# kaylode/vehicle-counting

Hardware: AMD Instinct MI355X
Metric: end-to-end frames/sec (detect+NMS+ReID+track), YOLOv5s 640px (higher is better)
Workload: dtype bf16; 1 GPU; YOLOv5s 640x640 single camera stream per GPU, bf16 convs (BASELINE.json configs[1]); workload_id=s640-bf16, clip_frames=512, objects=12, num_classes=80, detection_injection=False, weights=seeded synthetic (no checkpoints available), streams=1, ranks=1, counts_allgather_via=vc_allgather_counts (RCCL, C ABI), tracked_rows=155352, tracker=device-resident (one kernel per batch, no host round trip per frame)

## Files before the change

### vehicle-counting_amd/csrc/bneck_fused.hip

```cpp
#include <algorithm>

#include "kernels.h"
#include "conv_launch.h"

namespace vc {

typedef float f32x4b __attribute__((ext_vector_type(4)));
typedef float f32x2b __attribute__((ext_vector_type(2)));
typedef __bf16 bf16x8b __attribute__((ext_vector_type(8)));
typedef __bf16 bf16x2b __attribute__((ext_vector_type(2)));
typedef unsigned int u32x2b __attribute__((ext_vector_type(2)));
union ChunkB { uint4 u; bf16x8b h; };

#define BN_TH 8
#define BN_TW 16
#define BN_RW (BN_TW + 2)
#define BN_NH ((BN_TH + 2) * BN_RW)
#define BN_NT ((BN_NH + 15) / 16)
#define BN_NP BN_NH
#define BN_NW 8
#define BN_PLANE (BN_NP * 64)

__device__ __forceinline__ int bn_addr(int px, int chunk) { return (px * 4 + (chunk ^ ((px >> 1) & 2))) * 16; }
__device__ __forceinline__ f32x2b bn_sigmoid2(f32x2b x) {
// ... 6 lines not shown
    const f32x2b d = (f32x2b){__builtin_amdgcn_exp2f(t.x), __builtin_amdgcn_exp2f(t.y)} + (f32x2b){1.0f, 1.0f};
    return x * (f32x2b){__builtin_amdgcn_rcpf(d.x), __builtin_amdgcn_rcpf(d.y)};
}

struct BnArgs {
    const uint4 *w1, *w2;
    const float *b1, *b2;
    int kw1, kw2;
    const uint16_t* x; int in_cs, in_co;
    uint16_t* y; int out_cs, out_co;
    int B, H, W, tiles_x, tiles_y, res;
    const uint4* w3; const float* b3; int kw3;
    const uint16_t* y2; int y2_cs;
    uint16_t* z; int z_cs, z_co;
    long long* dbg;
};

template <bool CV3>
__global__ __launch_bounds__(BN_NW * 64) void bneck_fused_kernel(const BnArgs a) {
    const bool RES = a.res != 0;
    if (a.dbg && threadIdx.x == 0) a.dbg[(size_t)blockIdx.x * 2] = wall_clock64();
    __shared__ uint4 bs[2][2 * BN_NP * 4];
    __shared__ uint4 w1s[2 * 4 * 64];
    __shared__ uint4 w2s[18 * 4 * 64];
    __shared__ uint4 w3s[CV3 ? 4 * 8 * 64 : 1];
    __shared__ float b3s[CV3 ? 128 : 4];
    static_assert(sizeof(bs) + sizeof(w1s) + sizeof(w2s) + sizeof(w3s) + sizeof(b3s) <= 160 * 1024, "static LDS of bneck_fused_kernel exceeds a CU's 160 KB");
    const int lane = threadIdx.x & 63, wave = threadIdx.x >> 6;
    const int col = lane & 15, kq = lane >> 4;
    constexpr int NT = BN_NW * 64;
    for (int i = threadIdx.x; i < 2 * 4 * 64; i += NT) {
        const int l = i & 63, ct = (i >> 6) & 3, s = i >> 8;
        w1s[i] = a.w1[(size_t)(ct * 16 + (l & 15)) * a.kw1 + 4 * s + (l >> 4)];
    }
    for (int i = threadIdx.x; i < 18 * 4 * 64; i += NT) {
        const int l = i & 63, ct = (i >> 6) & 3, s = i >> 8;
        w2s[i] = a.w2[(size_t)(ct * 16 + (l & 15)) * a.kw2 + 4 * s + (l >> 4)];
    }
    if constexpr (CV3) {
        for (int i = threadIdx.x; i < 4 * 8 * 64; i += NT) {
            const int l = i & 63, ct = (i >> 6) & 7, s = i >> 9;
            w3s[i] = a.w3[(size_t)(ct * 16 + (l & 15)) * a.kw3 + 4 * s + (l >> 4)];
        }
        if (threadIdx.x < 128) b3s[threadIdx.x] = a.b3[threadIdx.x];
    }
    const bool producer = wave >= 4;
    const int gw = wave & 3;
    float4 bv[4];
#pragma unroll
    for (int ct = 0; ct < 4; ++ct) bv[ct] = *(const float4*)((producer ? a.b1 : a.b2) + ct * 16 + kq * 4);
    const int ntiles = a.B * a.tiles_y * a.tiles_x;
    const int nk = (int)blockIdx.x < ntiles ? (ntiles - 1 - (int)blockIdx.x) / (int)gridDim.x + 1 : 0;
    const bool odd = (kq & 1) != 0;
    __syncthreads();

    uint4 yf[3][2], yn[3][2];
    auto load_y = [&](int t, uint4 (&dst)[3][2]) {
        const int tx = t % a.tiles_x, ty = (t / a.tiles_x) % a.tiles_y, b = t / (a.tiles_x * a.tiles_y);
#pragma unroll
        for (int j = 0; j < 3; ++j) {
            const int n = (gw * 3 + j) * 16 + col;
            const int ry = (n * 3641) >> 16, rx = n - ry * BN_RW;
            const int gy = ty * BN_TH - 1 + ry, gx = tx * BN_TW - 1 + rx;
            dst[j][0] = make_uint4(0u, 0u, 0u, 0u); dst[j][1] = dst[j][0];
            if (n < BN_NH && gy >= 0 && gy < a.H && gx >= 0 && gx < a.W) {
                const uint16_t* px = a.x + (((size_t)b * a.H + gy) * a.W + gx) * a.in_cs + a.in_co + kq * 8;
                dst[j][0] = *(const uint4*)px; dst[j][1] = *(const uint4*)(px + 32);
            }
        }
    };
    if (producer && nk > 0) load_y(blockIdx.x, yf);
    for (int k = 0; k <= nk; ++k) {
        if (producer) {
            if (k < nk) {
                const int t = blockIdx.x + k * gridDim.x;
                if (k + 1 < nk) load_y(t + gridDim.x, yn);
                const int tx = t % a.tiles_x, ty = (t / a.tiles_x) % a.tiles_y;
                char* bsb = (char*)bs[k & 1];
                f32x4b pacc[3][4];
#pragma unroll
                for (int j = 0; j < 3; ++j) {
                    ChunkB y0f, y1f;
                    y0f.u = yf[j][0]; y1f.u = yf[j][1];
#pragma unroll
                    for (int ct = 0; ct < 4; ++ct) {
                        ChunkB w0, w1;
                        w0.u = w1s[(0 * 4 + ct) * 64 + lane]; w1.u = w1s[(1 * 4 + ct) * 64 + lane];
                        pacc[j][ct] = __builtin_amdgcn_mfma_f32_16x16x32_bf16(w0.h, y0f.h, (f32x4b){0.f, 0.f, 0.f, 0.f}, 0, 0, 0);
                        pacc[j][ct] = __builtin_amdgcn_mfma_f32_16x16x32_bf16(w1.h, y1f.h, pacc[j][ct], 0, 0, 0);
                    }
                }
// ... 7 lines not shown
#pragma unroll
                    for (int ct = 0; ct < 4; ++ct) {
                        const f32x4b acc = pacc[j][ct];
                        const f32x2b lo = bn_silu2((f32x2b){acc[0], acc[1]} + (f32x2b){bv[ct].x, bv[ct].y});
                        const f32x2b hi = bn_silu2((f32x2b){acc[2], acc[3]} + (f32x2b){bv[ct].z, bv[ct].w});
                        const bf16x2b p0 = {(__bf16)lo.x, (__bf16)lo.y}, p1 = {(__bf16)hi.x, (__bf16)hi.y};
                        uint2 v = make_uint2(__builtin_bit_cast(uint32_t, p0), __builtin_bit_cast(uint32_t, p1));
                        if (!inimg) v = make_uint2(0u, 0u);
                        if (n < BN_NH) *(uint2*)(bsb + (ct >> 1) * BN_PLANE + bn_addr(n, (ct & 1) * 2 + (kq >> 1)) + (kq & 1) * 8) = v;
                    }
                }
#pragma unroll
                for (int j = 0; j < 3; ++j) { yf[j][0] = yn[j][0]; yf[j][1] = yn[j][1]; }
            }
        } else if (k >= 1) {
            const int t = blockIdx.x + (k - 1) * gridDim.x;
            const int tx = t % a.tiles_x, ty = (t / a.tiles_x) % a.tiles_y, b = t / (a.tiles_x * a.tiles_y);
            const int oy0 = ty * BN_TH, ox0 = tx * BN_TW;
            const char* bsb = (const char*)bs[(k - 1) & 1];
            uint2 rs[4][2] = {};
            if (RES) {
#pragma unroll
                for (int q = 0; q < 2; ++q) {
                    const int oy = oy0 + gw * 2 + q, ox = ox0 + col;
                    const bool ok = oy < a.H && ox < a.W;
                    const uint16_t* px = a.x + (((size_t)b * a.H + min(oy, a.H - 1)) * a.W + min(ox, a.W - 1)) * a.in_cs + a.in_co + kq * 4;
#pragma unroll
                    for (int ct = 0; ct < 4; ++ct) rs[ct][q] = ok ? *(const uint2*)(px + ct * 16) : make_uint2(0u, 0u);
                }
            }
            uint4 y2f[2][2];
// ... 112 lines not shown
                    for (int q = 0; q < 2; ++q) {
                        const f32x2b lo = bn_silu2((f32x2b){zacc[ct][q][0], zacc[ct][q][1]} + (f32x2b){b3.x, b3.y});
                        const f32x2b hi = bn_silu2((f32x2b){zacc[ct][q][2], zacc[ct][q][3]} + (f32x2b){b3.z, b3.w});
                        const bf16x2b p0 = {(__bf16)lo.x, (__bf16)lo.y}, p1 = {(__bf16)hi.x, (__bf16)hi.y};
                        P[q] = make_uint2(__builtin_bit_cast(uint32_t, p0), __builtin_bit_cast(uint32_t, p1));
                    }
                    const u32x2b sx = __builtin_amdgcn_permlane16_swap(P[0].x, P[1].x, false, false);
                    const u32x2b sy = __builtin_amdgcn_permlane16_swap(P[0].y, P[1].y, false, false);
                    const uint4 o4 = make_uint4(sx.x, sy.x, sx.y, sy.y);
                    const int oy = oy0 + gw * 2 + (odd ? 1 : 0), ox = ox0 + col;
                    if (oy < a.H && ox < a.W)
                        *(uint4*)(a.z + (((size_t)b * a.H + oy) * a.W + ox) * a.z_cs + a.z_co + ct * 16 + (kq & ~1) * 4) = o4;
                }
            }
        }
        __syncthreads();
    }
    if (a.dbg && threadIdx.x == 0) a.dbg[(size_t)blockIdx.x * 2 + 1] = wall_clock64();
}

bool bneck_fused_applicable(const ConvP& pm1, const ConvP& pm2) {
    if (!(pm1.prec == PREC_BF16 && pm1.kh == 1 && pm1.kw == 1 && pm1.sh == 1 && pm1.sw == 1 && pm1.ph == 0 && pm1.pw == 0 && pm1.Cin == 64 && pm1.Cout == 64 &&
          pm1.act == ACT_SILU && pm1.res_mode == RES_NONE && !pm1.out_f32 && pm1.split == 0))
        return false;
    if (!(pm2.prec == PREC_BF16 && pm2.kh == 3 && pm2.kw == 3 && pm2.sh == 1 && pm2.sw == 1 && pm2.ph == 1 && pm2.pw == 1 && pm2.Cin == 64 && pm2.Cout == 64 &&
          pm2.act == ACT_SILU && (pm2.res_mode == RES_NONE || pm2.res_mode == RES_AFTER_ACT) && !pm2.out_f32 && pm2.split == 0))
        return false;
    if (!(pm2.in == pm1.out && pm2.in_co == pm1.out_co && pm2.in_cs == pm1.out_cs && pm2.H == pm1.H && pm2.W == pm1.W && pm2.B == pm1.B)) return false;
    if (pm2.res_mode == RES_AFTER_ACT && !(pm2.res == pm1.in && pm2.res_co == pm1.in_co && pm2.res_cs == pm1.in_cs)) return false;
    if (pm2.out == pm1.in && pm2.out_co < pm1.in_co + 64 && pm1.in_co < pm2.out_co + 64) return false;
    return pm1.in_cs % 8 == 0 && pm1.in_co % 8 == 0 && pm2.out_cs % 8 == 0 && pm2.out_co % 8 == 0 && pm1.Kp >= 64 && pm2.Kp >= 576;
}
// ... 23 lines not shown
    a.y = nullptr;
    a.w3 = (const uint4*)p3.w; a.b3 = p3.bias; a.kw3 = p3.Kp / 8;
    a.y2 = (const uint16_t*)p3.in + p3.in_co + 64; a.y2_cs = p3.in_cs;
    a.z = (uint16_t*)p3.out; a.z_cs = p3.out_cs; a.z_co = p3.out_co;
    a.B = pm1.B; a.H = pm1.H; a.W = pm1.W;
    a.tiles_x = (a.W + BN_TW - 1) / BN_TW; a.tiles_y = (a.H + BN_TH - 1) / BN_TH;
    const int ntiles = a.B * a.tiles_x * a.tiles_y;
    int dev = 0, cus = 256;
    hipDeviceProp_t prop;
    if (hipGetDevice(&dev) == hipSuccess && hipGetDeviceProperties(&prop, dev) == hipSuccess) cus = prop.multiProcessorCount;
    a.res = pm2.res_mode == RES_AFTER_ACT ? 1 : 0;
    int grid = std::min(ntiles, bneck_grid_cap(cus));
    if (grid_cap > 0) grid = std::min(grid, grid_cap);
    static WgStamps stamps("VC_BN_DBG", "bneck cv3", 1024, 2, 0, 1);
    a.dbg = stamps.next(grid, ntiles, s);
    launch_timed(pm1, bneck_fused_kernel<true>, dim3(grid), dim3(BN_NW * 64), 0, s, a);
    VC_HIP(hipGetLastError());
    if (a.dbg) stamps.report(s, [](const long long*, int, int) {});
    return VC_OK;
}

int launch_bneck_fused(const ConvP& pm1, const ConvP& pm2, hipStream_t s, int grid_cap) {
    if (!bneck_fused_applicable(pm1, pm2)) return VC_ERR_ARG;
    BnArgs a{};
    a.w1 = (const uint4*)pm1.w; a.w2 = (const uint4*)pm2.w; a.b1 = pm1.bias; a.b2 = pm2.bias;
    a.kw1 = pm1.Kp / 8; a.kw2 = pm2.Kp / 8;
    a.x = (const uint16_t*)pm1.in; a.in_cs = pm1.in_cs; a.in_co = pm1.in_co;
    a.y = (uint16_t*)pm2.out; a.out_cs = pm2.out_cs; a.out_co = pm2.out_co;
    a.B = pm1.B; a.H = pm1.H; a.W = pm1.W;
    a.tiles_x = (a.W + BN_TW - 1) / BN_TW; a.tiles_y = (a.H + BN_TH - 1) / BN_TH;
    const int ntiles = a.B * a.tiles_x * a.tiles_y;
    static const int cus = [] {
        int dev = 0, n = 256;
        hipDeviceProp_t prop;
        if (hipGetDevice(&dev) == hipSuccess && hipGetDeviceProperties(&prop, dev) == hipSuccess) n = prop.multiProcessorCount;
        return n;
    }();
    int grid = std::min(ntiles, bneck_grid_cap(cus));
    if (grid_cap > 0) grid = std::min(grid, grid_cap);
    a.res = pm2.res_mode == RES_AFTER_ACT ? 1 : 0;
    static WgStamps stamps("VC_BN_DBG", "bneck", 1024, 2, 0, 1);
    a.dbg = stamps.next(grid, ntiles, s);
    launch_timed(pm1, bneck_fused_kernel<false>, dim3(grid), dim3(BN_NW * 64), 0, s, a);
    VC_HIP(hipGetLastError());
    if (a.dbg) stamps.report(s, [](const long long*, int, int) {});
    return VC_OK;
}

}
```

### vehicle-counting_amd/csrc/c3_fused.hip

```cpp
#include <algorithm>

#include "kernels.h"
#include "conv_launch.h"

namespace vc {

typedef float f32x4c __attribute__((ext_vector_type(4)));
typedef float f32x2c __attribute__((ext_vector_type(2)));
typedef __bf16 bf16x8c __attribute__((ext_vector_type(8)));
typedef __bf16 bf16x2c __attribute__((ext_vector_type(2)));
typedef unsigned int u32x2c __attribute__((ext_vector_type(2)));
union ChunkC { uint4 u; bf16x8c h; };

#define C3_TH 8
#define C3_TW 16
#define C3_RW (C3_TW + 2)
#define C3_NH ((C3_TH + 2) * C3_RW)
#define C3_NT ((C3_NH + 15) / 16)
#define C3_NP (C3_NT * 16)
#define C3_NW 4

__device__ __forceinline__ int c3_addr(int px, int chunk) { return (px * 4 + (chunk ^ ((px >> 1) & 2))) * 16; }
__device__ __forceinline__ f32x2c c3_silu2(f32x2c x) {
    const f32x2c t = x * (f32x2c){-1.442695040888963387f, -1.442695040888963387f};
// ... 6 lines not shown
    f32x2c hi = (f32x2c){a[2], a[3]} + (f32x2c){b.z, b.w};
    if constexpr (!NOTRANS) { lo = c3_silu2(lo); hi = c3_silu2(hi); }
    const bf16x2c p0 = {(__bf16)lo.x, (__bf16)lo.y}, p1 = {(__bf16)hi.x, (__bf16)hi.y};
    return make_uint2(__builtin_bit_cast(uint32_t, p0), __builtin_bit_cast(uint32_t, p1));
}

struct C3Args {
    const uint4 *w12, *wm1, *wm2, *w3;
    const float *b12, *bm1, *bm2, *b3;
    int kw12, kwm1, kwm2, kw3;
    const uint16_t* x; int in_cs, in_co;
    uint16_t* y; int out_cs, out_co;
    int B, H, W, tiles_x, tiles_y;
    int abl;
    long long* dbg;
};

template <bool DIAG>
__global__ __launch_bounds__(C3_NW * 64, 2) void c3_fused_kernel(const C3Args a) {
    const int abl = DIAG ? a.abl : 0;
    if (a.dbg && threadIdx.x == 0) a.dbg[(size_t)blockIdx.x * 2] = wall_clock64();
    __shared__ uint4 xa[2 * C3_NP * 4];
    __shared__ uint4 yb[C3_NP * 4];
    __shared__ uint4 yc[C3_TH * C3_TW * 4];
    __shared__ uint4 w12s[2 * 4 * 64], wm1s[2 * 64], wm2s[9 * 2 * 64], w3s[2 * 4 * 64];
    const int lane = threadIdx.x & 63, wave = threadIdx.x >> 6;
    const int col = lane & 15, kq = lane >> 4;
    constexpr int NT = C3_NW * 64;
    for (int i = threadIdx.x; i < 2 * 4 * 64; i += NT) {
        const int l = i & 63, ct = (i >> 6) & 3, s = i >> 8;
// ... 24 lines not shown
#pragma unroll
        for (int k = 0; k < NPRE; ++k) {
            const int i = threadIdx.x + k * NT;
            const int n = i >> 3, c = i & 7;
            const int ry = (n * 3641) >> 16, rx = n - ry * C3_RW;
            const int gy = y0 + ry, gx = x0 + rx;
            pre[k] = make_uint4(0u, 0u, 0u, 0u);
            if (n < C3_NH && gy >= 0 && gy < a.H && gx >= 0 && gx < a.W && !(abl & 2))
                pre[k] = *(const uint4*)(a.x + (((size_t)b * a.H + gy) * a.W + gx) * a.in_cs + a.in_co + c * 8);
        }
    };
    char* xab = (char*)xa;
    char* ybb = (char*)yb;
    char* ycb = (char*)yc;
    const bool odd = (kq & 1) != 0;
    if ((int)blockIdx.x < ntiles) fetch(blockIdx.x);
    for (int t = blockIdx.x; t < ntiles; t += gridDim.x) {
        const int tx = t % a.tiles_x, ty = (t / a.tiles_x) % a.tiles_y, b = t / (a.tiles_x * a.tiles_y);
        const int oy0 = ty * C3_TH, ox0 = tx * C3_TW;
#pragma unroll
        for (int k = 0; k < NPRE; ++k) {
            const int i = threadIdx.x + k * NT;
            const int n = i >> 3, c = i & 7;
            if (n < C3_NH) *(uint4*)(xab + (c >> 2) * (C3_NP * 64) + c3_addr(n, c & 3)) = pre[k];
        }
        __syncthreads();
        if (t + (int)gridDim.x < ntiles) fetch(t + gridDim.x);

        for (int pt = wave; pt < C3_NT && !(abl & 16); pt += C3_NW) {
            const int n = pt * 16 + col;
            ChunkC x0f, x1f;
            x0f.u = *(const uint4*)(xab + c3_addr(n, kq));
            x1f.u = *(const uint4*)(xab + C3_NP * 64 + c3_addr(n, kq));
            f32x4c acc[4];
#pragma unroll
            for (int ct = 0; ct < 4; ++ct) {
                ChunkC w0, w1;
                w0.u = w12s[(0 * 4 + ct) * 64 + lane]; w1.u = w12s[(1 * 4 + ct) * 64 + lane];
                acc[ct] = __builtin_amdgcn_mfma_f32_16x16x32_bf16(w0.h, x0f.h, (f32x4c){0.f, 0.f, 0.f, 0.f}, 0, 0, 0);
                acc[ct] = __builtin_amdgcn_mfma_f32_16x16x32_bf16(w1.h, x1f.h, acc[ct], 0, 0, 0);
            }
            const int ry = (n * 3641) >> 16, rx = n - ry * C3_RW;
// ... 86 lines not shown
                    acc[ct][q] = __builtin_amdgcn_mfma_f32_16x16x32_bf16(w1.h, yf[q].h, acc[ct][q], 0, 0, 0);
                }
            }
#pragma unroll
            for (int ct = 0; ct < 4; ++ct) {
                const uint2 P0 = act4(acc[ct][0], b3[ct]), P1 = act4(acc[ct][1], b3[ct]);
                const u32x2c sx = __builtin_amdgcn_permlane16_swap(P0.x, P1.x, false, false);
                const u32x2c sy = __builtin_amdgcn_permlane16_swap(P0.y, P1.y, false, false);
                const uint4 o4 = make_uint4(sx.x, sy.x, sx.y, sy.y);
                const int oy = oy0 + wave * 2 + (odd ? 1 : 0), ox = ox0 + col;
                if (oy < a.H && ox < a.W && !(abl & 4))
                    *(uint4*)(a.y + (((size_t)b * a.H + oy) * a.W + ox) * a.out_cs + a.out_co + ct * 16 + (kq & ~1) * 4) = o4;
            }
        }
    }
    if (a.dbg && threadIdx.x == 0) a.dbg[(size_t)blockIdx.x * 2 + 1] = wall_clock64();
}

bool c3_fused_applicable(const ConvP& p12, const ConvP& pm1, const ConvP& pm2, const ConvP& p3) {
    auto pw = [](const ConvP& p, int cin, int cout) {
        return p.prec == PREC_BF16 && p.kh == 1 && p.kw == 1 && p.sh == 1 && p.sw == 1 && p.ph == 0 && p.pw == 0 && p.Cin == cin && p.Cout == cout &&
               p.act == ACT_SILU && p.res_mode == RES_NONE && !p.out_f32;
    };
    if (!pw(p12, 64, 64) || p12.split != 32 || !pw(pm1, 32, 32) || pm1.split != 0 || !pw(p3, 64, 64) || p3.split != 0) return false;
    if (!(pm2.prec == PREC_BF16 && pm2.kh == 3 && pm2.kw == 3 && pm2.sh == 1 && pm2.sw == 1 && pm2.ph == 1 && pm2.pw == 1 && pm2.Cin == 32 && pm2.Cout == 32 &&
          pm2.act == ACT_SILU && pm2.res_mode == RES_AFTER_ACT && !pm2.out_f32 && pm2.split == 0))
        return false;
    const bool chain = pm1.in == p12.out && pm1.in_co == p12.out_co && pm2.in == pm1.out && pm2.in_co == pm1.out_co && pm2.res == p12.out && pm2.res_co == p12.out_co &&
                       pm2.out == p3.in && pm2.out_co == p3.in_co && p12.out2 == p3.in && p12.out2_co == p3.in_co + 32 && pm2.out_cs == p3.in_cs && p12.out2_cs == p3.in_cs;
    const bool shape = pm1.H == p12.H && pm2.H == p12.H && p3.H == p12.H && pm1.W == p12.W && pm2.W == p12.W && p3.W == p12.W && pm1.B == p12.B && p3.B == p12.B;
// ... 2 lines not shown

int launch_c3_fused(const ConvP& p12, const ConvP& pm1, const ConvP& pm2, const ConvP& p3, hipStream_t s, int grid_cap) {
    if (!c3_fused_applicable(p12, pm1, pm2, p3)) return VC_ERR_ARG;
    C3Args a{};
    a.w12 = (const uint4*)p12.w; a.wm1 = (const uint4*)pm1.w; a.wm2 = (const uint4*)pm2.w; a.w3 = (const uint4*)p3.w;
    a.b12 = p12.bias; a.bm1 = pm1.bias; a.bm2 = pm2.bias; a.b3 = p3.bias;
    a.kw12 = p12.Kp / 8; a.kwm1 = pm1.Kp / 8; a.kwm2 = pm2.Kp / 8; a.kw3 = p3.Kp / 8;
    a.x = (const uint16_t*)p12.in; a.in_cs = p12.in_cs; a.in_co = p12.in_co;
    a.y = (uint16_t*)p3.out; a.out_cs = p3.out_cs; a.out_co = p3.out_co;
    a.B = p12.B; a.H = p12.H; a.W = p12.W;
    a.tiles_x = (a.W + C3_TW - 1) / C3_TW; a.tiles_y = (a.H + C3_TH - 1) / C3_TH;
    const int ntiles = a.B * a.tiles_x * a.tiles_y;
    static const int slots_hw = resident_workgroups(c3_fused_kernel<false>, C3_NW * 64);
    int grid = std::min(ntiles, std::max(256, slots_hw - conv_slots_reserve() / 2));
    if (grid_cap > 0) grid = std::min(grid, grid_cap);
    a.abl = p12.ablate;
    static WgStamps stamps("VC_C3_DBG", "c3", 1024, 2, 0, 1);
    a.dbg = stamps.next(grid, ntiles, s);
    if (a.abl) launch_timed(p12, c3_fused_kernel<true>, dim3(grid), dim3(C3_NW * 64), 0, s, a);
    else launch_timed(p12, c3_fused_kernel<false>, dim3(grid), dim3(C3_NW * 64), 0, s, a);
    VC_HIP(hipGetLastError());
    if (a.dbg) stamps.report(s, [](const long long*, int, int) {});
    return VC_OK;
}

}
```

### vehicle-counting_amd/csrc/engine.h

```cpp
#pragma once
#include <chrono>
#include <condition_variable>
#include <deque>
#include <map>
#include <mutex>
#include <memory>
#include <string>
#include <vector>

#include "kernels.h"
#include "det_prep.h"
#include "host_stage.h"

namespace vc {

struct ConvParam {
    std::string name;
    int O = 0, I = 0, kh = 0, kw = 0;
    bool set = false;
    bool pair_stem = false;
    int fuse_a = -1, fuse_b = -1;
    int obj_of = -1;
    bool hidden = false;
    std::vector<float> w, b;
// ... 79 lines not shown
}

struct vc_render;

struct vc_engine {
    vc_engine_config cfg{};
    int prec = 0;
    int aux_prec = 0;
    float act_scale = 1.0f;
    hipStream_t stream = nullptr;
    hipStream_t dstream = nullptr;
    hipStream_t rstream = nullptr;
    hipStream_t hstream = nullptr;
    hipEvent_t ev_fork = nullptr, ev_join = nullptr;
    static constexpr unsigned kTileCtrPairs = 1024;
    unsigned* d_tile_ctr = nullptr;
    unsigned tile_ctr_seq = 0;
    unsigned tile_ctr_ring = kTileCtrPairs;
    int conv_slots = 0;
    void* d_zero = nullptr; size_t zero_bytes = 0; bool want_hc_count = false;
    hipEvent_t ev_det[2] = {nullptr, nullptr};
    hipEvent_t ev_reid[3] = {nullptr, nullptr, nullptr};
    bool finalized = false;
    struct Options { int c3_fused = 1, bneck_fused = 1, bneck_cv3 = 1, front_fused = 1, crop_per_pixel = 0, sparse_head = 1, ff_ablate = 0, c3_ablate = 0, reid_block_fused = 1, dyn_tiles = 1, head_side = 1, fuse_upsample = 1, sppf_sep = 1, fuse_s2_pw = 1, stem_direct = 1, embed_kept_only = 1; } opt;
    std::vector<void*> allocs;
    std::vector<void*> host_allocs;

    vc::Net yolo;
    int ch[5] = {0, 0, 0, 0, 0}, rep[4] = {0, 0, 0, 0};
    std::map<std::string, vc::View> ybuf;
    const vc::YoloPlan* last_plan = nullptr;
    std::vector<vc::ConvP> s2pw_folded;
    std::vector<std::pair<vc::View, vc::View>> up_folded;
    std::map<std::vector<int>, vc::YoloPlan> yolo_plans;
    std::map<std::pair<int, int>, vc::ReidPlan> reid_plans;
    uint8_t* d_frames = nullptr;
    size_t d_frames_bytes = 0;
    float* d_logits[3] = {nullptr, nullptr, nullptr};
    void* d_obj[3] = {nullptr, nullptr, nullptr};
// ... 116 lines not shown
    vc::ProfCat prof[VC_PROF_NCAT];
    hipEvent_t ev0 = nullptr, ev1 = nullptr;
    std::map<std::string, int> tuned;
    bool tuned_dirty = false;
    std::string op_log;
    double last_ms = 0;

    std::vector<float> inject_det;
    std::vector<int> inject_count;
    int inject_b = 0, inject_n = 0;
};

namespace vc {
int pack_and_upload(std::vector<void*>& allocs, ConvParam& p, int prec, float act_scale = 1.0f);
inline int dev_alloc(vc_engine* e, void** p, size_t bytes) { return dev_alloc(e->allocs, p, bytes); }
inline unsigned* tile_ctr_next(vc_engine* e) {
    if (!e->d_tile_ctr || !e->opt.dyn_tiles) return nullptr;
    return e->d_tile_ctr + (size_t)(e->tile_ctr_seq++ % e->tile_ctr_ring) * 16;
}
int dev_realloc(vc_engine* e, void** p, size_t bytes);
int host_alloc(vc_engine* e, void** p, size_t bytes);
inline int round_up(int x, int m) { return (x + m - 1) / m * m; }
extern const float kAnchors[3][6];
void yolo_define(vc_engine* e);
int yolo_alloc(vc_engine* e);
int yolo_build_ops(vc_engine* e, int B, int Hn, int Wn, bool sparse, YoloPlan& plan);
void reid_define(vc_engine* e);
int reid_alloc(vc_engine* e);
int reid_build_ops(vc_engine* e, int k0, int k, ReidPlan& plan);
int reid_cpad(int prec);
View mkview(const View& buf, int B, int H, int W, int C, int co);
struct ConvSlice { void* ptr; int cs, co; };
// ... 48 lines not shown
```

### vehicle-counting_amd/csrc/engine.hip

```cpp
#include <algorithm>
#include <cmath>
#include <cstdarg>
#include <cstdlib>

#include "engine.h"

namespace vc {

static thread_local char g_err[1024] = "";
void set_error(const char* fmt, ...) {
    va_list ap;
    va_start(ap, fmt);
    vsnprintf(g_err, sizeof(g_err), fmt, ap);
    va_end(ap);
}
const char* last_error() { return g_err; }

int dev_alloc(std::vector<void*>& allocs, void** p, size_t bytes) {
    if (bytes == 0) bytes = 16;
    VC_HIP(hipMalloc(p, bytes));
    allocs.push_back(*p);
    return VC_OK;
}
int dev_realloc(vc_engine* e, void** p, size_t bytes) {
// ... 130 lines not shown
    int ndev = 0;
    VC_HIP(hipGetDeviceCount(&ndev));
    VC_CHECK(cfg->device >= 0 && cfg->device < ndev, VC_ERR_HIP, "device %d not present (%d visible)", cfg->device, ndev);
    VC_HIP(hipSetDevice(cfg->device));
    vc_engine* e = new vc_engine();
    e->cfg = *cfg;
    e->prec = cfg->precision;
    e->aux_prec = cfg->precision == VC_PREC_FP8 ? (int)PREC_BF16 : cfg->precision;
    e->act_scale = getenv("VC_FP8_ACT_SCALE") ? (float)atof(getenv("VC_FP8_ACT_SCALE")) : 1.0f;
    {
        auto env_int = [](const char* name, int dflt) { const char* v = getenv(name); return v ? atoi(v) : dflt; };
        e->opt.c3_fused = env_int("VC_C3_FUSED", 1); e->opt.bneck_fused = env_int("VC_BNECK_FUSED", 1); e->opt.bneck_cv3 = env_int("VC_BNECK_CV3", 1);
        e->opt.front_fused = env_int("VC_FRONT_FUSED", 1); e->opt.crop_per_pixel = getenv("VC_CROP_PER_PIXEL") ? 1 : 0;
        e->opt.sparse_head = env_int("VC_SPARSE_HEAD", 1); e->opt.reid_block_fused = env_int("VC_REID_BLOCK_FUSED", 1); e->opt.head_side = env_int("VC_HEAD_SIDE", 1); e->opt.fuse_upsample = env_int("VC_FUSE_UPSAMPLE", 1); e->opt.sppf_sep = env_int("VC_SPPF_SEP", 1); e->opt.fuse_s2_pw = env_int("VC_FUSE_S2PW", 1);
        e->opt.embed_kept_only = env_int("VC_EMBED_KEPT_ONLY", 1);
        e->opt.dyn_tiles = env_int("VC_DYN_TILES", 1);
        e->conv_slots = env_int("VC_CONV_SLOTS", 0);
        e->tile_ctr_ring = (unsigned)std::min(std::max(env_int("VC_DYN_TILES_RING", (int)vc_engine::kTileCtrPairs), 1), (int)vc_engine::kTileCtrPairs);
    }
    memcpy(e->anchors, kAnchors, sizeof(kAnchors));
    int st = VC_OK;
    do {
        int plo = 0, phi = 0;
        hipDeviceGetStreamPriorityRange(&plo, &phi);
        const int reserve = getenv("VC_TRACK_CUS") ? atoi(getenv("VC_TRACK_CUS")) : 0;
        bool ok;
        if (reserve > 0) {
            hipDeviceProp_t prop;
            hipGetDeviceProperties(&prop, cfg->device);
            const int ncu = prop.multiProcessorCount, words = (ncu + 31) / 32;
            std::vector<uint32_t> mt(words, 0), mc(words, 0);
// ... 155 lines not shown
}

int vc_engine_set_option(vc_engine* e, const char* name, int value) {
    VC_CHECK(e && name, VC_ERR_ARG, "null argument");
    const std::string n = name;
    if (n == "embed_kept_only") { e->opt.embed_kept_only = value; return VC_OK; }
    if (n == "c3_fused") e->opt.c3_fused = value;
    else if (n == "bneck_fused") e->opt.bneck_fused = value;
    else if (n == "bneck_cv3") e->opt.bneck_cv3 = value;
    else if (n == "front_fused") e->opt.front_fused = value;
    else if (n == "crop_per_pixel") e->opt.crop_per_pixel = value;
    else if (n == "sparse_head") e->opt.sparse_head = value;
    else if (n == "reid_block_fused") e->opt.reid_block_fused = value;
    else if (n == "dyn_tiles_ring") { VC_CHECK(value >= 1 && value <= (int)vc_engine::kTileCtrPairs, VC_ERR_ARG, "dyn_tiles_ring must be 1 .. %u", vc_engine::kTileCtrPairs); e->tile_ctr_ring = (unsigned)value; return VC_OK; }
    else if (n == "dyn_tiles") e->opt.dyn_tiles = value;
    else if (n == "head_side") e->opt.head_side = value;
    else if (n == "fuse_upsample") e->opt.fuse_upsample = value;
    else if (n == "sppf_sep") e->opt.sppf_sep = value;
    else if (n == "fuse_s2_pw") e->opt.fuse_s2_pw = value;
    else if (n == "stem_direct") e->opt.stem_direct = value;
    else if (n == "ff_ablate") e->opt.ff_ablate = value;
    else if (n == "c3_ablate") e->opt.c3_ablate = value;
    else if (n == "dot_arena_mb") { VC_CHECK(value >= 0, VC_ERR_ARG, "dot_arena_mb must be >= 0"); e->dot_arena_max_floats = (size_t)value * 262144; }
    else { set_error("unknown option '%s'", name); return VC_ERR_NOTFOUND; }
    plans_retune(e);
    return VC_OK;
}

int vc_tune_export(vc_engine* e, char* buf, size_t cap, size_t* size) {
    VC_CHECK(e && size, VC_ERR_ARG, "null argument");
// ... 262 lines not shown
```

### vehicle-counting_amd/csrc/engine_run.hip

```cpp
#include <algorithm>
#include <cmath>
#include <cstdlib>

#include "engine.h"

namespace vc {

static std::string tune_key(const ConvP& c) {
    int bucket = 1;
    while (bucket < c.M) bucket <<= 1;
    char k[160];
    snprintf(k, sizeof(k), "p%d_ci%d_co%d_k%dx%d_s%d_h%d_w%d_K%d_m%d_sp%d%s", c.prec, c.Cin, c.Cout, c.kh, c.kw, c.sh, c.H, c.W, c.K, bucket, c.split,
             c.in_up ? "_up" : "");
    return k;
}

static std::mutex g_tune_mu;
static std::map<std::string, int> g_tuned;

void tune_cache_load(vc_engine* e) {
    const char* path = getenv("VC_TUNE_CACHE");
    if (!path) return;
    FILE* f = fopen(path, "r");
    if (!f) return;
// ... 106 lines not shown
    };

    const bool front_ok = e->opt.front_fused > 0 && o1 && front_fused_applicable(cp, o1->conv);
    c.u8_src = e->stem_src && cp.in == e->ybuf["in"].ptr;
    const bool stem_ok = e->opt.stem_direct != 0 && stem_direct_applicable(cp);
    if (c.u8_src && !((stem_ok && stem_u8_applicable(cp, e->stem_geom)) || (front_ok && front_fused_resize_ok(e->stem_geom)))) {
        ProfScope ps(e, VC_PROF_DETECT_AUX, 0, 0, c.s);
        VC_TRY(launch_letterbox(e->stem_src, e->ybuf["in"].ptr, cp.B, e->stem_geom, e->aux_prec, c.s));
        e->stem_src = nullptr; e->in_stale = false;
        c.u8_src = false;
    }
    if (e->opt.c3_fused != 0 && o1 && o2 && o3 && c3_fused_applicable(cp, o1->conv, o2->conv, o3->conv)) {
        fused(103, 4, fl + conv_flops(*o1) + conv_flops(*o2) + conv_flops(*o3),
              in_bytes + w_bytes(op) + w_bytes(*o1) + w_bytes(*o2) + w_bytes(*o3) + out_bytes(*o3), 64, 64, 1, 1);
        cp.ablate = e->opt.c3_ablate;
        L.launch = [](ConvCtx& x) { return launch_c3_fused(x.cp, x.op[1].conv, x.op[2].conv, x.op[3].conv, x.s); };
    } else if (e->opt.reid_block_fused != 0 && o1 && reid_block_fused_applicable(cp, o1->conv)) {
        fused(106, 2, fl + conv_flops(*o1), in_bytes + w_bytes(op) + w_bytes(*o1) + out_bytes(*o1), 64, 1152, 3, 1);
        L.launch = [](ConvCtx& x) { return launch_reid_block_fused(x.cp, x.op[1].conv, x.s); };
    } else if (e->opt.bneck_fused != 0 && e->opt.bneck_cv3 != 0 && o1 && o2 && bneck_cv3_fused_applicable(cp, o1->conv, o2->conv)) {
        fused(105, 3, fl + conv_flops(*o1) + conv_flops(*o2),
              (double)cp.B * cp.H * cp.W * (cp.Cin + 64) * es + w_bytes(op) + w_bytes(*o1) + w_bytes(*o2) + out_bytes(*o2), 128, 768, 3, 1);
        L.launch = [](ConvCtx& x) { return launch_bneck_cv3_fused(x.cp, x.op[1].conv, x.op[2].conv, x.s); };
    } else if (e->opt.bneck_fused != 0 && o1 && bneck_fused_applicable(cp, o1->conv)) {
        fused(104, 2, fl + conv_flops(*o1), in_bytes + w_bytes(op) + w_bytes(*o1) + out_bytes(*o1), 64, 640, 3, 1);
        L.launch = [](ConvCtx& x) { return launch_bneck_fused(x.cp, x.op[1].conv, x.s); };
    } else if (e->opt.fuse_s2_pw != 0 && op.sole_reader_next && o1 && s2halo_pw_applicable(cp, o1->conv)) {
        fused(107, 2, fl + conv_flops(*o1), in_bytes + w_bytes(op) + w_bytes(*o1) + out_bytes(*o1), 128, cp.K + 128, 3, 2);
        L.launch = [](ConvCtx& x) {
            VC_TRY(launch_s2halo_pw(x.cp, x.op[1].conv, x.s));
            static const bool also_store = getenv("VC_S2PW_STORE") && atoi(getenv("VC_S2PW_STORE")) != 0;
            if (!also_store) x.e->s2pw_folded.push_back(x.op->conv);
            return (int)VC_OK;
        };
    } else if (front_ok && (e->opt.front_fused == 2 || c.u8_src)) {
        L.cfg = 102; L.n_ops = 2; L.flops = fl + conv_flops(*o1); L.bytes = in_bytes + w_bytes(op) + w_bytes(*o1) + out_bytes(*o1);
        cp.ablate = e->opt.ff_ablate;
        cp.slots = e->conv_slots; cp.tile_ctr = tile_ctr_next(e);
        L.launch = [](ConvCtx& x) {
            VC_TRY(launch_front_fused(x.cp, x.op[1].conv, x.u8_src ? x.e->stem_src : nullptr, x.e->stem_geom, x.s));
            x.e->l0_stale = true;
            return (int)VC_OK;
        };
    } else if (stem_ok) {
        L.cfg = 100;
        if (nx && nx->kind == Op::TO_FP8 && nx->a.ptr == cp.out && nx->a.co == cp.out_co) { c.q8 = &nx->b; L.n_ops = 2; }
        L.launch = [](ConvCtx& x) {
            return x.u8_src ? launch_stem_direct_u8(x.cp, x.e->stem_src, x.e->stem_geom, x.s, x.q8, 1.0f / x.e->act_scale)
                            : launch_stem_direct(x.cp, x.s, x.q8, 1.0f / x.e->act_scale);
        };
    } else if (nx && nx->kind == Op::MAXPOOL && nx->a.ptr == cp.out && reid_stem_applicable(cp, nx->b.cs, nx->b.co)) {
        L.cfg = 101; L.n_ops = 2;
        L.launch = [](ConvCtx& x) { return launch_reid_stem_pool(x.cp, x.op[1].b.ptr, x.s); };
// ... 260 lines not shown
```

### vehicle-counting_amd/csrc/vc_common.h

```cpp
#pragma once
#include <hip/hip_runtime.h>
#include <hip/hip_ext.h>
#include <cmath>
#include <cstdint>
#include <cstdio>
#include <cstring>
#include <string>

#include "../../include/vcount_hip.h"

namespace vc {

void set_error(const char* fmt, ...);
const char* last_error();

#define VC_HIP(expr)                                                                            \
    do {                                                                                        \
        hipError_t _e = (expr);                                                                 \
        if (_e != hipSuccess) {                                                                 \
            vc::set_error("%s:%d %s -> %s", __FILE__, __LINE__, #expr, hipGetErrorString(_e));  \
            return VC_ERR_HIP;                                                                  \
        }                                                                                       \
    } while (0)

// ... 123 lines not shown
    int up_C, up_cs, up_co;
    int ksplit;
    float* sk_ws;
    int* sk_tickets;
    long long* dbg;
    int s2_th, s2_tw;
    int slots;
    int ablate;
    unsigned* tile_ctr;
};

#if defined(__HIPCC__)
__device__ __forceinline__ int tile_claim(unsigned* ctr) {
    return (int)gridDim.x + (int)__hip_atomic_fetch_add(ctr, 1u, __ATOMIC_RELAXED, __HIP_MEMORY_SCOPE_AGENT);
}
__device__ __forceinline__ void tile_claims_done(unsigned* ctr) {
    if (__hip_atomic_fetch_add(ctr + 1, 1u, __ATOMIC_RELAXED, __HIP_MEMORY_SCOPE_AGENT) == gridDim.x - 1) {
        __hip_atomic_store(ctr, 0u, __ATOMIC_RELAXED, __HIP_MEMORY_SCOPE_AGENT);
        __hip_atomic_store(ctr + 1, 0u, __ATOMIC_RELAXED, __HIP_MEMORY_SCOPE_AGENT);
    }
}
#endif

template <class K, class... A>
static inline void launch_timed(const ConvP& p, K kernel, dim3 grid, dim3 block, unsigned lds, hipStream_t s, A... args) {
    if (p.ev_start) hipExtLaunchKernelGGL(kernel, grid, block, lds, s, p.ev_start, p.ev_stop, 0, args...);
    else hipLaunchKernelGGL(kernel, grid, block, lds, s, args...);
}

int launch_conv(const ConvP& p, hipStream_t s);
// ... 34 lines not shown
```

Measured before the change: 23400 frames/s.

## Add chunked dynamic tile claiming to fused bottleneck and C3 kernels

Extends atomic-counter dynamic tile scheduling, previously used only in the front fused kernel, to the fused bottleneck (with and without cv3) and C3 kernels. Tiles after the first wave are handed out in power-of-two chunks of decreasing size, to cut atomic traffic while still balancing the tail. The bottleneck kernel gets a walker thread that fills a small LDS tile queue ahead of the producer and consumer waves. A per-kernel mask option selects which kernels use it. This adds atomics and queue bookkeeping per tile and changes loop termination, in exchange for less load imbalance across workgroups.

```diff
diff --git a/vehicle-counting_amd/csrc/bneck_fused.hip b/vehicle-counting_amd/csrc/bneck_fused.hip
--- a/vehicle-counting_amd/csrc/bneck_fused.hip
+++ b/vehicle-counting_amd/csrc/bneck_fused.hip
@@ -2,6 +2,7 @@
 
 #include "kernels.h"
 #include "conv_launch.h"
+#include "tile_sched.h"
 
 namespace vc {
 
@@ -44,6 +45,7 @@
     const uint16_t* y2; int y2_cs;
     uint16_t* z; int z_cs, z_co;
     long long* dbg;
+    unsigned* ctr;
 };
 
 template <bool CV3>
@@ -55,7 +57,8 @@
     __shared__ uint4 w2s[18 * 4 * 64];
     __shared__ uint4 w3s[CV3 ? 4 * 8 * 64 : 1];
     __shared__ float b3s[CV3 ? 128 : 4];
-    static_assert(sizeof(bs) + sizeof(w1s) + sizeof(w2s) + sizeof(w3s) + sizeof(b3s) <= 160 * 1024, "static LDS of bneck_fused_kernel exceeds a CU's 160 KB");
+    __shared__ int tq[4];
+    static_assert(sizeof(bs) + sizeof(w1s) + sizeof(w2s) + sizeof(w3s) + sizeof(b3s) + sizeof(tq) <= 160 * 1024, "static LDS of bneck_fused_kernel exceeds a CU's 160 KB");
     const int lane = threadIdx.x & 63, wave = threadIdx.x >> 6;
     const int col = lane & 15, kq = lane >> 4;
     constexpr int NT = BN_NW * 64;
@@ -80,8 +83,23 @@
 #pragma unroll
     for (int ct = 0; ct < 4; ++ct) bv[ct] = *(const float4*)((producer ? a.b1 : a.b2) + ct * 16 + kq * 4);
     const int ntiles = a.B * a.tiles_y * a.tiles_x;
-    const int nk = (int)blockIdx.x < ntiles ? (ntiles - 1 - (int)blockIdx.x) / (int)gridDim.x + 1 : 0;
     const bool odd = (kq & 1) != 0;
+    unsigned* const ctr = a.ctr;
+    const bool walker = threadIdx.x == 4 * 64;
+    int w_cur = 0, w_left = 0, w_pend = 0;
+    if (walker) {
+        const int t0 = (int)blockIdx.x < ntiles ? (int)blockIdx.x : ntiles;
+        tq[0] = t0;
+        if (ctr) {
+            int len;
+            w_cur = tile_chunk(tile_claim_chunk(ctr), ntiles, (int)gridDim.x, &len);
+            w_left = len - 1;
+            if (w_cur < ntiles && w_left == 0) w_pend = tile_claim_chunk(ctr);
+        } else {
+            w_cur = t0 < ntiles - (int)gridDim.x ? t0 + (int)gridDim.x : ntiles;
+        }
+        tq[1] = w_cur;
+    }
     __syncthreads();
 
     uint4 yf[3][2], yn[3][2];
@@ -99,12 +117,29 @@
             }
         }
     };
-    if (producer && nk > 0) load_y(blockIdx.x, yf);
-    for (int k = 0; k <= nk; ++k) {
+    if (producer && (int)blockIdx.x < ntiles) load_y(blockIdx.x, yf);
+    for (int k = 0;; ++k) {
+        const int tk = __builtin_amdgcn_readfirstlane(tq[k & 3]);
         if (producer) {
-            if (k < nk) {
-                const int t = blockIdx.x + k * gridDim.x;
-                if (k + 1 < nk) load_y(t + gridDim.x, yn);
+            if (tk < ntiles) {
+                const int t = tk;
+                const int t1 = __builtin_amdgcn_readfirstlane(tq[(k + 1) & 3]);
+                if (walker) {
+                    int nx = ntiles;
+                    if (w_cur < ntiles) {
+                        if (!ctr) nx = w_cur < ntiles - (int)gridDim.x ? w_cur + (int)gridDim.x : ntiles;
+                        else if (w_left > 0) { nx = w_cur + 1; --w_left; }
+                        else {
+                            int len;
+                            nx = tile_chunk(w_pend, ntiles, (int)gridDim.x, &len);
+                            w_left = len - 1;
+                        }
+                        if (ctr && nx < ntiles && w_left == 0) w_pend = tile_claim_chunk(ctr);
+                    }
+                    tq[(k + 2) & 3] = nx;
+                    w_cur = nx;
+                }
+                if (t1 < ntiles) load_y(t1, yn);
                 const int tx = t % a.tiles_x, ty = (t / a.tiles_x) % a.tiles_y;
                 char* bsb = (char*)bs[k & 1];
                 f32x4b pacc[3][4];
@@ -142,7 +177,7 @@
                 for (int j = 0; j < 3; ++j) { yf[j][0] = yn[j][0]; yf[j][1] = yn[j][1]; }
             }
         } else if (k >= 1) {
-            const int t = blockIdx.x + (k - 1) * gridDim.x;
+            const int t = __builtin_amdgcn_readfirstlane(tq[(k - 1) & 3]);
             const int tx = t % a.tiles_x, ty = (t / a.tiles_x) % a.tiles_y, b = t / (a.tiles_x * a.tiles_y);
             const int oy0 = ty * BN_TH, ox0 = tx * BN_TW;
             const char* bsb = (const char*)bs[(k - 1) & 1];
@@ -285,8 +320,10 @@
                 }
             }
         }
+        if (tk >= ntiles) break;
         __syncthreads();
     }
+    if (ctr && walker) tile_claims_done(ctr);
     if (a.dbg && threadIdx.x == 0) a.dbg[(size_t)blockIdx.x * 2 + 1] = wall_clock64();
 }
 
@@ -340,6 +377,7 @@
     if (grid_cap > 0) grid = std::min(grid, grid_cap);
     static WgStamps stamps("VC_BN_DBG", "bneck cv3", 1024, 2, 0, 1);
     a.dbg = stamps.next(grid, ntiles, s);
+    a.ctr = pm1.tile_ctr;
     launch_timed(pm1, bneck_fused_kernel<true>, dim3(grid), dim3(BN_NW * 64), 0, s, a);
     VC_HIP(hipGetLastError());
     if (a.dbg) stamps.report(s, [](const long long*, int, int) {});
@@ -367,6 +405,7 @@
     a.res = pm2.res_mode == RES_AFTER_ACT ? 1 : 0;
     static WgStamps stamps("VC_BN_DBG", "bneck", 1024, 2, 0, 1);
     a.dbg = stamps.next(grid, ntiles, s);
+    a.ctr = pm1.tile_ctr;
     launch_timed(pm1, bneck_fused_kernel<false>, dim3(grid), dim3(BN_NW * 64), 0, s, a);
     VC_HIP(hipGetLastError());
     if (a.dbg) stamps.report(s, [](const long long*, int, int) {});
diff --git a/vehicle-counting_amd/csrc/c3_fused.hip b/vehicle-counting_amd/csrc/c3_fused.hip
--- a/vehicle-counting_amd/csrc/c3_fused.hip
+++ b/vehicle-counting_amd/csrc/c3_fused.hip
@@ -2,6 +2,7 @@
 
 #include "kernels.h"
 #include "conv_launch.h"
+#include "tile_sched.h"
 
 namespace vc {
 
@@ -44,6 +45,7 @@
     int B, H, W, tiles_x, tiles_y;
     int abl;
     long long* dbg;
+    unsigned* ctr;
 };
 
 template <bool DIAG>
@@ -98,8 +100,13 @@
     char* ybb = (char*)yb;
     char* ycb = (char*)yc;
     const bool odd = (kq & 1) != 0;
+    unsigned* const ctr = a.ctr;
+    int* const nxt_s = (int*)(ybb + (C3_NP - 1) * 64);
+    int pend = 0;
+    if (ctr && threadIdx.x == 0) pend = tile_claim_chunk(ctr);
     if ((int)blockIdx.x < ntiles) fetch(blockIdx.x);
-    for (int t = blockIdx.x; t < ntiles; t += gridDim.x) {
+    int left = 0, tn;
+    for (int t = blockIdx.x; t < ntiles; t = tn) {
         const int tx = t % a.tiles_x, ty = (t / a.tiles_x) % a.tiles_y, b = t / (a.tiles_x * a.tiles_y);
         const int oy0 = ty * C3_TH, ox0 = tx * C3_TW;
 #pragma unroll
@@ -108,8 +115,19 @@
             const int n = i >> 3, c = i & 7;
             if (n < C3_NH) *(uint4*)(xab + (c >> 2) * (C3_NP * 64) + c3_addr(n, c & 3)) = pre[k];
         }
-        __syncthreads();
-        if (t + (int)gridDim.x < ntiles) fetch(t + gridDim.x);
+        if (ctr && left == 0 && threadIdx.x == 0) {
+            int len;
+            nxt_s[0] = tile_chunk(pend, ntiles, (int)gridDim.x, &len);
+            nxt_s[1] = len;
+        }
+        __syncthreads();
+        if (!ctr) tn = t + (int)gridDim.x;
+        else if (left > 0) { tn = t + 1; --left; }
+        else { tn = nxt_s[0]; left = nxt_s[1] - 1; }
+        if (tn < ntiles) {
+            fetch(tn);
+            if (ctr && left == 0 && threadIdx.x == 0) pend = tile_claim_chunk(ctr);
+        }
 
         for (int pt = wave; pt < C3_NT && !(abl & 16); pt += C3_NW) {
             const int n = pt * 16 + col;
@@ -226,6 +244,7 @@
             }
         }
     }
+    if (ctr && threadIdx.x == 0) tile_claims_done(ctr);
     if (a.dbg && threadIdx.x == 0) a.dbg[(size_t)blockIdx.x * 2 + 1] = wall_clock64();
 }
 
@@ -258,6 +277,8 @@
     static const int slots_hw = resident_workgroups(c3_fused_kernel<false>, C3_NW * 64);
     int grid = std::min(ntiles, std::max(256, slots_hw - conv_slots_reserve() / 2));
     if (grid_cap > 0) grid = std::min(grid, grid_cap);
+    else if (p12.slots > 0) grid = std::min(grid, p12.slots);
+    a.ctr = p12.tile_ctr;
     a.abl = p12.ablate;
     static WgStamps stamps("VC_C3_DBG", "c3", 1024, 2, 0, 1);
     a.dbg = stamps.next(grid, ntiles, s);
diff --git a/vehicle-counting_amd/csrc/engine.h b/vehicle-counting_amd/csrc/engine.h
--- a/vehicle-counting_amd/csrc/engine.h
+++ b/vehicle-counting_amd/csrc/engine.h
@@ -117,6 +117,7 @@
     hipStream_t hstream = nullptr;
     hipEvent_t ev_fork = nullptr, ev_join = nullptr;
     static constexpr unsigned kTileCtrPairs = 1024;
+    static constexpr int kDynTilesKept = 7;
     unsigned* d_tile_ctr = nullptr;
     unsigned tile_ctr_seq = 0;
     unsigned tile_ctr_ring = kTileCtrPairs;
@@ -125,7 +126,7 @@
     hipEvent_t ev_det[2] = {nullptr, nullptr};
     hipEvent_t ev_reid[3] = {nullptr, nullptr, nullptr};
     bool finalized = false;
-    struct Options { int c3_fused = 1, bneck_fused = 1, bneck_cv3 = 1, front_fused = 1, crop_per_pixel = 0, sparse_head = 1, ff_ablate = 0, c3_ablate = 0, reid_block_fused = 1, dyn_tiles = 1, head_side = 1, fuse_upsample = 1, sppf_sep = 1, fuse_s2_pw = 1, stem_direct = 1, embed_kept_only = 1; } opt;
+    struct Options { int c3_fused = 1, bneck_fused = 1, bneck_cv3 = 1, front_fused = 1, crop_per_pixel = 0, sparse_head = 1, ff_ablate = 0, c3_ablate = 0, reid_block_fused = 1, dyn_tiles = 1, dyn_tiles_mask = kDynTilesKept, head_side = 1, fuse_upsample = 1, sppf_sep = 1, fuse_s2_pw = 1, stem_direct = 1, embed_kept_only = 1; } opt;
     std::vector<void*> allocs;
     std::vector<void*> host_allocs;
 
@@ -272,8 +273,8 @@
 namespace vc {
 int pack_and_upload(std::vector<void*>& allocs, ConvParam& p, int prec, float act_scale = 1.0f);
 inline int dev_alloc(vc_engine* e, void** p, size_t bytes) { return dev_alloc(e->allocs, p, bytes); }
-inline unsigned* tile_ctr_next(vc_engine* e) {
-    if (!e->d_tile_ctr || !e->opt.dyn_tiles) return nullptr;
+inline unsigned* tile_ctr_next(vc_engine* e, int bit) {
+    if (!e->d_tile_ctr || !e->opt.dyn_tiles || !(e->opt.dyn_tiles_mask & bit)) return nullptr;
     return e->d_tile_ctr + (size_t)(e->tile_ctr_seq++ % e->tile_ctr_ring) * 16;
 }
 int dev_realloc(vc_engine* e, void** p, size_t bytes);
diff --git a/vehicle-counting_amd/csrc/engine.hip b/vehicle-counting_amd/csrc/engine.hip
--- a/vehicle-counting_amd/csrc/engine.hip
+++ b/vehicle-counting_amd/csrc/engine.hip
@@ -168,7 +168,7 @@
         e->opt.front_fused = env_int("VC_FRONT_FUSED", 1); e->opt.crop_per_pixel = getenv("VC_CROP_PER_PIXEL") ? 1 : 0;
         e->opt.sparse_head = env_int("VC_SPARSE_HEAD", 1); e->opt.reid_block_fused = env_int("VC_REID_BLOCK_FUSED", 1); e->opt.head_side = env_int("VC_HEAD_SIDE", 1); e->opt.fuse_upsample = env_int("VC_FUSE_UPSAMPLE", 1); e->opt.sppf_sep = env_int("VC_SPPF_SEP", 1); e->opt.fuse_s2_pw = env_int("VC_FUSE_S2PW", 1);
         e->opt.embed_kept_only = env_int("VC_EMBED_KEPT_ONLY", 1);
-        e->opt.dyn_tiles = env_int("VC_DYN_TILES", 1);
+        e->opt.dyn_tiles = env_int("VC_DYN_TILES", 1); e->opt.dyn_tiles_mask = env_int("VC_DYN_TILES_MASK", vc_engine::kDynTilesKept);
         e->conv_slots = env_int("VC_CONV_SLOTS", 0);
         e->tile_ctr_ring = (unsigned)std::min(std::max(env_int("VC_DYN_TILES_RING", (int)vc_engine::kTileCtrPairs), 1), (int)vc_engine::kTileCtrPairs);
     }
@@ -354,6 +354,7 @@
     else if (n == "reid_block_fused") e->opt.reid_block_fused = value;
     else if (n == "dyn_tiles_ring") { VC_CHECK(value >= 1 && value <= (int)vc_engine::kTileCtrPairs, VC_ERR_ARG, "dyn_tiles_ring must be 1 .. %u", vc_engine::kTileCtrPairs); e->tile_ctr_ring = (unsigned)value; return VC_OK; }
     else if (n == "dyn_tiles") e->opt.dyn_tiles = value;
+    else if (n == "dyn_tiles_mask") e->opt.dyn_tiles_mask = value;
     else if (n == "head_side") e->opt.head_side = value;
     else if (n == "fuse_upsample") e->opt.fuse_upsample = value;
     else if (n == "sppf_sep") e->opt.sppf_sep = value;
diff --git a/vehicle-counting_amd/csrc/engine_run.hip b/vehicle-counting_amd/csrc/engine_run.hip
--- a/vehicle-counting_amd/csrc/engine_run.hip
+++ b/vehicle-counting_amd/csrc/engine_run.hip
@@ -144,6 +144,7 @@
         fused(103, 4, fl + conv_flops(*o1) + conv_flops(*o2) + conv_flops(*o3),
               in_bytes + w_bytes(op) + w_bytes(*o1) + w_bytes(*o2) + w_bytes(*o3) + out_bytes(*o3), 64, 64, 1, 1);
         cp.ablate = e->opt.c3_ablate;
+        cp.slots = e->conv_slots; cp.tile_ctr = tile_ctr_next(e, 2);
         L.launch = [](ConvCtx& x) { return launch_c3_fused(x.cp, x.op[1].conv, x.op[2].conv, x.op[3].conv, x.s); };
     } else if (e->opt.reid_block_fused != 0 && o1 && reid_block_fused_applicable(cp, o1->conv)) {
         fused(106, 2, fl + conv_flops(*o1), in_bytes + w_bytes(op) + w_bytes(*o1) + out_bytes(*o1), 64, 1152, 3, 1);
@@ -151,9 +152,11 @@
     } else if (e->opt.bneck_fused != 0 && e->opt.bneck_cv3 != 0 && o1 && o2 && bneck_cv3_fused_applicable(cp, o1->conv, o2->conv)) {
         fused(105, 3, fl + conv_flops(*o1) + conv_flops(*o2),
               (double)cp.B * cp.H * cp.W * (cp.Cin + 64) * es + w_bytes(op) + w_bytes(*o1) + w_bytes(*o2) + out_bytes(*o2), 128, 768, 3, 1);
+        cp.tile_ctr = tile_ctr_next(e, 4);
         L.launch = [](ConvCtx& x) { return launch_bneck_cv3_fused(x.cp, x.op[1].conv, x.op[2].conv, x.s); };
     } else if (e->opt.bneck_fused != 0 && o1 && bneck_fused_applicable(cp, o1->conv)) {
         fused(104, 2, fl + conv_flops(*o1), in_bytes + w_bytes(op) + w_bytes(*o1) + out_bytes(*o1), 64, 640, 3, 1);
+        cp.tile_ctr = tile_ctr_next(e, 4);
         L.launch = [](ConvCtx& x) { return launch_bneck_fused(x.cp, x.op[1].conv, x.s); };
     } else if (e->opt.fuse_s2_pw != 0 && op.sole_reader_next && o1 && s2halo_pw_applicable(cp, o1->conv)) {
         fused(107, 2, fl + conv_flops(*o1), in_bytes + w_bytes(op) + w_bytes(*o1) + out_bytes(*o1), 128, cp.K + 128, 3, 2);
@@ -166,7 +169,7 @@
     } else if (front_ok && (e->opt.front_fused == 2 || c.u8_src)) {
         L.cfg = 102; L.n_ops = 2; L.flops = fl + conv_flops(*o1); L.bytes = in_bytes + w_bytes(op) + w_bytes(*o1) + out_bytes(*o1);
         cp.ablate = e->opt.ff_ablate;
-        cp.slots = e->conv_slots; cp.tile_ctr = tile_ctr_next(e);
+        cp.slots = e->conv_slots; cp.tile_ctr = tile_ctr_next(e, 1);
         L.launch = [](ConvCtx& x) {
             VC_TRY(launch_front_fused(x.cp, x.op[1].conv, x.u8_src ? x.e->stem_src : nullptr, x.e->stem_geom, x.s));
             x.e->l0_stale = true;
diff --git a/vehicle-counting_amd/csrc/tile_sched.h b/vehicle-counting_amd/csrc/tile_sched.h
--- /dev/null
+++ b/vehicle-counting_amd/csrc/tile_sched.h
@@ -0,0 +1,49 @@
+#pragma once
+
+#if defined(__HIPCC__)
+#define VC_HD __host__ __device__
+#else
+#define VC_HD
+#endif
+
+namespace vc {
+
+#define TILE_CHUNK_LOG2 3
+#define TILE_CHUNK_MAX (1 << TILE_CHUNK_LOG2)
+
+struct TileChunkCounts { int n[TILE_CHUNK_LOG2 + 1]; };
+
+VC_HD static inline TileChunkCounts tile_chunk_counts(int ntiles, int grid) {
+    TileChunkCounts c;
+    int rest = ntiles > grid ? ntiles - grid : 0;
+    for (int k = 0; k < TILE_CHUNK_LOG2; ++k) {
+        const int m = rest >> k < grid ? rest >> k : grid;
+        c.n[k] = m;
+        rest -= m << k;
+    }
+    c.n[TILE_CHUNK_LOG2] = rest >> TILE_CHUNK_LOG2;
+    rest -= c.n[TILE_CHUNK_LOG2] << TILE_CHUNK_LOG2;
+    for (int k = 0; k < TILE_CHUNK_LOG2; ++k) c.n[k] += (rest >> k) & 1;
+    return c;
+}
+
+VC_HD static inline int tile_chunk_count(int ntiles, int grid) {
+    const TileChunkCounts c = tile_chunk_counts(ntiles, grid);
+    int s = 0;
+    for (int k = 0; k <= TILE_CHUNK_LOG2; ++k) s += c.n[k];
+    return s;
+}
+
+VC_HD static inline int tile_chunk(int chunk, int ntiles, int grid, int* len) {
+    const TileChunkCounts c = tile_chunk_counts(ntiles, grid);
+    int first = grid;
+    for (int k = TILE_CHUNK_LOG2; k >= 0; --k) {
+        if (chunk < c.n[k]) { *len = 1 << k; return first + (chunk << k); }
+        chunk -= c.n[k];
+        first += c.n[k] << k;
+    }
+    *len = 0;
+    return ntiles;
+}
+
+}
diff --git a/vehicle-counting_amd/csrc/vc_common.h b/vehicle-counting_amd/csrc/vc_common.h
--- a/vehicle-counting_amd/csrc/vc_common.h
+++ b/vehicle-counting_amd/csrc/vc_common.h
@@ -161,6 +161,9 @@
 __device__ __forceinline__ int tile_claim(unsigned* ctr) {
     return (int)gridDim.x + (int)__hip_atomic_fetch_add(ctr, 1u, __ATOMIC_RELAXED, __HIP_MEMORY_SCOPE_AGENT);
 }
+__device__ __forceinline__ int tile_claim_chunk(unsigned* ctr) {
+    return (int)__hip_atomic_fetch_add(ctr, 1u, __ATOMIC_RELAXED, __HIP_MEMORY_SCOPE_AGENT);
+}
 __device__ __forceinline__ void tile_claims_done(unsigned* ctr) {
     if (__hip_atomic_fetch_add(ctr + 1, 1u, __ATOMIC_RELAXED, __HIP_MEMORY_SCOPE_AGENT) == gridDim.x - 1) {
         __hip_atomic_store(ctr, 0u, __ATOMIC_RELAXED, __HIP_MEMORY_SCOPE_AGENT);
```

New measurement: 23930 frames/s (median of 6 runs). 2.3% higher.
